# lordnn/OF_DIS

Measured on AMD Instinct MI355X. Metric: MPix/s (and frames/sec) 1080p op-point-2; avg EPE vs CPU ref, higher is better.
Workload: dtype f32; 1 GPU; run_OF_INT 1920x1080 op-point 2, 4096 pairs/GPU/step; width=1920, height=1080, channels=1, oppoint=2, batch_per_gpu=4096, streams=2, pairs_per_launch=2048, parallelism=frame-sharded x1

## Files before the change

### of_dis_amd/csrc/ofdis_internal.h

```cpp
#pragma once

#include <hip/hip_runtime.h>
#include <stdint.h>

namespace ofdis {

struct LevelGeom {
  int w, h;
  int pad;
  int W, H;
  int nopw, noph, npatch, offw, offh;
  float tmp_lb, tmp_ubw, tmp_ubh;
  int level;
};

struct PyrBaseArgs {
  const uint8_t *img_a, *img_b;
  int n, W0, H0, noc;
  int padl, padt;
  int log2s;
  int w, h;
  float *out;
  int rgb_sad;
};

struct PyrGradmagArgs {
  const uint8_t *img_a, *img_b;
  int n, W0, H0, padl, padt, Wp, Hp;
  float *out;
};

struct PyrDownArgs {
  const float *src;
  float *dst;
  int n2, w, h, noc;
};

struct PyrPadGradArgs {
  const float *lvl;
  float *img, *dx, *dy;
  int n2, w, h, noc, pad;
  int per_value;
};

struct PatchArgs {
  const float *img_a, *dx_a, *dy_a, *img_b;
  const float *prev;
  long prev_frame_stride;
  int prev_comp_stride, prev_elem_stride, prev_w;
  float *p_iter;
  float *pweight;
  int n, nop, noc, p, novals, steps;
  int costfct, patnorm, max_iter, min_iter;
  float dp_thresh_sq, dr_thresh, res_thresh, outlierthresh;
  float outlier_sq;
  int camlr;
  int wave_per_patch;
  int generic;
  int window;
  int quad;
  int x16;
  int absw;
  int aslots;
  int buf32;
  int fdiv;
  int maxres;
  int stage;
  LevelGeom g;
};

struct AggArgs {
  const float *p_iter, *pweight;
  const float *cg_p_iter, *cg_pweight;
  float *flow;
  int n, nop, noc, p, novals, steps;
  int absw;
  int aslots;
  int stage;
  LevelGeom g;
};

struct TvArgs {
  const float *img_a, *img_b;
  float *flow;
  float *wxs, *wys;
  float *du, *dv, *mask, *s;
  float *coef;
  float *t, *dt;
  float *Ix, *Iy, *Iz, *Ixx, *Ixy, *Iyy, *Ixz, *Iyz;
  long sp;
  int wrap;
  int skew_slots;
  int n, nop, noc, w, h, pad, W;
  float quarter_alpha, hdo3, hgo3, omega;
  int first_iter;
  int solverit;
  int camlr;
  int sor_generic;
  int sor_variant;
  int sor_point;
  int sor_cring;
  int sor_rows2;
  int smsys;
  int prepd;
  int smsys2d;
  int smsys_prefetch;
  int smsys_small;
  int smsys_march;
  int smsys_deriv;
  int prepd_df;
  int sor_redblack;
  int lat;
};

struct UpArgs {
  const float *flow;
  float *out;
  int n, nop, wl, hl, log2s, W0, H0, offx, offy;
  int nt_store;
  int form;
};

struct InitArgs {
  const float *init;
  float *out;
  int n, nop, W0, H0, padl, padt, log2k, wo, ho;
  float sc, scale;
};

struct FbArgs {
  const float *fw, *bw;
  uint8_t *occ_fw, *occ_bw;
  float *err_fw, *err_bw;
  int n, W, H;
  float alpha, beta;
};

void launch_fb_check(const FbArgs &a, hipStream_t s);
void launch_init_area(const InitArgs &a, hipStream_t s);
void warm_kernels_module(hipStream_t s);
void warm_tvrb_module(hipStream_t s);
void launch_pyr_base(const PyrBaseArgs &a, hipStream_t s);
void launch_pyr_gradmag(const PyrGradmagArgs &a, hipStream_t s);
void launch_pyr_down(const PyrDownArgs &a, hipStream_t s);
void launch_pyr_pad_grad(const PyrPadGradArgs &a, hipStream_t s);
bool launch_patch(const PatchArgs &a, hipStream_t s);
void launch_aggregate(const AggArgs &a, hipStream_t s);
void launch_tv_prep(const TvArgs &a, hipStream_t s);
void launch_tv_deriv1(const TvArgs &a, hipStream_t s);
void launch_tv_deriv2(const TvArgs &a, hipStream_t s);
bool tv_prepd_ok(const TvArgs &a);
void launch_tv_prepd(const TvArgs &a, hipStream_t s);
void launch_tv_smooth(const TvArgs &a, hipStream_t s);
void launch_tv_system(const TvArgs &a, hipStream_t s);
bool tv_smsys_ok(const TvArgs &a);
bool tv_deriv_fused(const TvArgs &a);
void launch_tv_smsys(const TvArgs &a, hipStream_t s);
void launch_tv_sor(const TvArgs &a, hipStream_t s);
bool tv_level_rb_ok(const TvArgs &a);
void launch_tv_level_rb(const TvArgs &a, int n_inner, hipStream_t s);
void launch_tv_final(const TvArgs &a, hipStream_t s);
void launch_upsample(const UpArgs &a, hipStream_t s);

}
```

### of_dis_amd/csrc/ofdis_kernels.hip

```cpp
#include "ofdis_internal.h"
#include "ofdis_math.h"

#include <algorithm>
#include <cstdlib>
#include <type_traits>
#include <utility>

#pragma clang fp contract(off)

namespace ofdis {
typedef float float4_u __attribute__((ext_vector_type(4), aligned(4)));
typedef float float4_v __attribute__((ext_vector_type(4)));

namespace {

#include "ofdis_tv_dev.inc"
#include "ofdis_agg_dev.inc"

inline unsigned ceil_div(long a, long b) { return (unsigned)((a + b - 1) / b); }

template <int V>
using Int = std::integral_constant<int, V>;
template <int... Vs, class F>
inline bool pick(int v, F &&f) {
// ... 3799 lines not shown
      hv[q][s] = nvv[s];
    }
    own_u[q] = cru;
    own_v[q] = crv;
    hsh[q] = csh;
    hsv[q] = csv;
    if (nw > 1) {
      const int par = t & 1;
      float rec[4 * NV4];
#pragma unroll
      for (int s = 0; s < S; ++s) { rec[s] = nu[s]; rec[S + s] = nvv[s]; }
      rec[2 * S] = csv;
#pragma unroll
      for (int k = 2 * S + 1; k < 4 * NV4; ++k) rec[k] = 0.0f;
      if (lane == 63) {
#pragma unroll
        for (int k = 0; k < NV4; ++k) xtop[par][wv][k] = make_float4(rec[4 * k], rec[4 * k + 1], rec[4 * k + 2], rec[4 * k + 3]);
      }
      if (lane == 0) {
#pragma unroll
        for (int k = 0; k < NV4; ++k) xbot[par][wv][k] = make_float4(rec[4 * k], rec[4 * k + 1], rec[4 * k + 2], rec[4 * k + 3]);
      }
      __syncthreads();
    }
  }

  template <int PH>
  __device__ __forceinline__ void steps(const int t) {
    step<PH>(t + PH);
    if constexpr (PH + 1 < U) steps<PH + 1>(t);
  }
};

template <int S, int MODE, int MAXT>
__global__ __launch_bounds__(MAXT) void k_tv_sor_pipe(TvArgs a) {
  using P = SorPipe<S, MODE>;
  __shared__ float4 xtop[2][16][P::NV4];
  __shared__ float4 xbot[2][16][P::NV4];
  P st;
  const int f = blockIdx.x;
  st.w = a.w;
  st.h = a.h;
  st.y = threadIdx.x;
  st.lane = st.y & 63;
  st.wv = st.y >> 6;
  st.nw = (int)(blockDim.x >> 6);
  const long fo = (long)f * a.sp;
  st.du = a.du + fo;
  st.dv = a.dv + fo;
  st.C = reinterpret_cast<const float4 *>(a.coef) + fo * (MODE == 0 ? 2 : 1);
  st.xtop = xtop;
  st.xbot = xbot;
  st.omega = a.omega;
  st.has_top = st.y > 0;
  st.has_bot = st.y < a.h - 1;
  st.notop = !st.has_top;
  st.border = !st.has_top || !st.has_bot;
  st.get_top = st.lane == 0 && st.wv > 0;
  st.get_bot = st.lane == 63 && st.wv < st.nw - 1;
  st.wrap = a.wrap;
  st.dump = (unsigned)(a.skew_slots + st.lane);
#pragma unroll
  for (int q = 0; q < 2; ++q) {
#pragma unroll
    for (int s = 0; s < S; ++s) st.hu[q][s] = st.hv[q][s] = 0.0f;
    st.own_u[q] = st.own_v[q] = st.hsh[q] = st.hsv[q] = 0.0f;
  }
  if (st.y == 0 && a.w > 0) {
    st.own_u[1] = st.du[0];
    if (MODE == 0) st.own_v[1] = st.dv[0];
  }
  const int T = (a.w - 1) + (a.h - 1) + 2 * (S - 1) + 1;
  const int TU = (T + P::U - 1) / P::U * P::U;
  st.load(0, st.L[0]);
  st.load(1, st.L[1]);
  for (int t = 0; t < TU; t += P::U) st.template steps<0>(t);
}

__device__ __forceinline__ int sor_row2(int d, int lim, int rmax) {
  const int dd = max(d, 0);
  return min(dd >= lim ? dd - lim : dd, rmax);
}

template <int S, int MODE, int SI, int NB, int CRN, int R = 1, bool SEL = false>
struct SorLane {
  static constexpr bool FIRST = SI == 0, LAST = SI == S - 1;
  static_assert(CRN == 0 || S <= 3, "coefficient ring depth 6 needs S <= 3");
  static constexpr int PD = NB - 1;
  static constexpr int U = NB % 3 == 0 ? (NB < 6 ? 6 : NB) : 3 * NB;
  static constexpr int CW = MODE == 0 ? 2 : 1;
  struct Ld {
    float4 c0[R], c1[R];
    f2v o[R], b[R];
  };
  Ld L0, L1, L2, L3, L4, L5;
  template <int I>
  __device__ __forceinline__ Ld &buf() {
    static_assert(I < NB && NB <= 6, "buffer index");
    if constexpr (I == 0) return L0;
    else if constexpr (I == 1) return L1;
    else if constexpr (I == 2) return L2;
    else if constexpr (I == 3) return L3;
    else if constexpr (I == 4) return L4;
    else return L5;
  }
  f2v pp[R];
  float phr[R];
  float pvv[R];
  f2v prv[R];
  static constexpr bool DPT = R == 1;
  bool top_lds;
  const float4 *C;
  const float *du_r, *dv_r;
  float *du, *dv;
  f2v *ring_s;
  const f2v *ring_p;
  float *sv_s;
  float4 *cr;
  int w, h, y, s, lim, rmax, hplane;
  unsigned yc[R];
  bool border[R], notop[R];
  float omega;
#ifdef OFDIS_SOR_PROBE
  unsigned *probe = nullptr;
#endif

  __device__ __forceinline__ void load(int t, Ld &B) {
    const int d = t - 2 * s;
    const unsigned r0 = (unsigned)sor_row2(d, lim, rmax) * (unsigned)hplane;
    const unsigned r1 = FIRST ? (unsigned)sor_row2(d + 1, lim, rmax) * (unsigned)hplane : 0u;
#pragma unroll
    for (int r = 0; r < R; ++r) {
      unsigned yr = yc[r];
      if (SEL) {
        const int lo = min(max(d - w + 1, 0), h - 1), hi = max(min(d, h - 1), 0);
        yr = (unsigned)min(max(y + 64 * r, lo), hi);
      }
      if (FIRST || CRN == 0) {
        const float4 *cp = C + (size_t)r0 * CW;
        B.c0[r] = cp[yr * CW];
        if (MODE == 0) B.c1[r] = cp[yr * CW + 1];
      }
      if (FIRST) {
        const float *u0 = du_r + r0, *u1 = du_r + r1;
        float ov = 0.0f, bv = 0.0f;
        if (MODE == 0) {
          const float *v0 = dv_r + r0, *v1 = dv_r + r1;
          ov = v0[yr];
          bv = v1[yr + 1];
        }
        B.o[r] = f2v{u0[yr], ov};
        B.b[r] = f2v{u1[yr + 1], bv};
      }
    }
  }

  template <int Q>
  __device__ __forceinline__ void step(const int t) {
    constexpr int m0 = Q % 3, m1 = (Q + 2) % 3;
#ifdef OFDIS_SOR_PROBE
    const unsigned pt0 = probe_clock();
    unsigned pt1 = 0, pt2 = 0;
#endif
    Ld &B = buf<Q % NB>();
    const Ld &Bn = buf<(Q + 1) % NB>();
    load(t + PD, buf<(Q + PD) % NB>());
    const int d = t - 2 * s;
#pragma unroll
    for (int r = 0; r < R; ++r) {
      constexpr int RO = 64 * 3;
      const int yr = y + 64 * r;
      const int xp = d - yr;
      const bool hasl = xp > 0, hasr = xp < w - 1;
      f2v o, rgt, bt;
      if (FIRST) {
        o = B.o[r]; rgt = Bn.o[r]; bt = B.b[r];
      } else {
        o = prv[r]; rgt = ring_p[r * RO + m1]; bt = ring_p[r * RO + 3 + m1];
        prv[r] = rgt;
      }
      constexpr int cs = ((Q - 2 * SI) % 6 + 6) % 6, ct = (cs + 5) % 6;
      float4 c0, c1;
      if (CRN > 0) {
        if (FIRST) {
          c0 = B.c0[r];
          c1 = MODE == 0 ? B.c1[r] : B.c0[r];
          cr[cs * CW * CRN + 64 * r] = c0;
          if (MODE == 0) cr[(cs * CW + 1) * CRN + 64 * r] = c1;
        } else {
          c0 = cr[cs * CW * CRN + 64 * r];
          c1 = MODE == 0 ? cr[(cs * CW + 1) * CRN + 64 * r] : c0;
        }
      } else {
        c0 = B.c0[r];
        c1 = MODE == 0 ? B.c1[r] : B.c0[r];
      }
      f2v tp;
      float tsv;
      if (DPT) {
        tp = f2v{dpp_from_prev_lane(pp[r].x), MODE == 0 ? dpp_from_prev_lane(pp[r].y) : 0.0f};
        tsv = dpp_from_prev_lane(pvv[r]);
        if (top_lds) {
          tp = ring_s[r * RO + m1 - 3];
          tsv = CRN > 0 ? cr[(ct * CW + CW - 1) * CRN - 1 + 64 * r].w : sv_s[r * RO + m1 - 3];
        }
      } else {
        tp = ring_s[r * RO + m1 - 3];
        tsv = CRN > 0 ? cr[(ct * CW + CW - 1) * CRN - 1 + 64 * r].w : sv_s[r * RO + m1 - 3];
      }
      f2v nw;
      float vv;
#ifdef OFDIS_SOR_PROBE
      {
        const float dep = ((c0.x + c1.x) + (tp.x + tsv)) + (rgt.x + bt.x);
        asm volatile("; probe use %0" ::"v"(dep) : "memory");
        pt1 = probe_clock();
      }
#endif
      if (MODE == 0) {
        const float hr = c1.z;
        vv = c1.w;
        const f2v bb = f2v{c1.x, c1.y};
        const f2v rr = hasr ? rgt : f2v{0.0f, 0.0f};
        const f2v X = hr * rr, Y = tsv * tp, Z = vv * bt;
        const f2v l = X + (border[r] ? bb : Y);
        const f2v rg = (border[r] ? f2v{-0.0f, -0.0f} : bb) + (border[r] ? (notop[r] ? Z : Y) : Z);
        const f2v sr = l + rg;
        const f2v Bv = hasl ? phr[r] * pp[r] + sr : sr;
        const f2v m_1 = f2v{c0.x, c0.y} * Bv.x, m_2 = f2v{c0.z, c0.w} * Bv.y;
        nw = o + omega * ((m_1 + m_2) - o);
        phr[r] = hr;
      } else {
        const float a11 = c0.x, b1 = c0.y, hr = c0.z;
        vv = c0.w;
        const bool has_top = !notop[r], has_bot = !(border[r] && has_top);
        const float tu = tp.x, ur = hasr ? rgt.x : 0.0f, hl = phr[r];
        float su = 0.0f;
        su = has_top ? su - tsv * tu : su;
        su = hasl ? su - hl * pp[r].x : su;
        su = has_bot ? su - vv * bt.x : su;
        su = hasr ? su - hr * ur : su;
        const float A = a11, Bq = b1 - su;
        nw = f2v{(1.0f - omega) * o.x + omega * (Bq / A), 0.0f};
        phr[r] = hr;
      }
      ring_s[r * RO + m0] = nw;
      if (CRN == 0) sv_s[r * RO + m0] = vv;
      pvv[r] = vv;
      if (LAST) {
        if ((unsigned)xp < (unsigned)w && yr < h) {
          const unsigned r0 = (unsigned)sor_row2(d, lim, rmax) * (unsigned)hplane;
          du[r0 + (unsigned)yr] = nw.x;
          if (MODE == 0) dv[r0 + (unsigned)yr] = nw.y;
        }
      }
      pp[r] = nw;
    }
#ifdef OFDIS_SOR_PROBE
    asm volatile("s_waitcnt lgkmcnt(0)" ::: "memory");
    pt2 = probe_clock();
#endif
    __syncthreads();
#ifdef OFDIS_SOR_PROBE
    if (probe && (threadIdx.x & 63) == 0 && t < 1024)
      *reinterpret_cast<uint4 *>(probe + 4 * t) = make_uint4(pt0, pt1, pt2, probe_clock());
#endif
  }

  template <int J>
  __device__ __forceinline__ void prologue(const int t) {
    load(t + J, buf<J>());
    if constexpr (J + 1 < PD) prologue<J + 1>(t);
  }
  template <int J>
  __device__ __forceinline__ void block(const int t) {
    step<J>(t + J);
    if constexpr (J + 1 < U) block<J + 1>(t);
  }

  __device__ __forceinline__ void run(int T, int y0, int ymax) {
#pragma unroll
    for (int r = 0; r < R; ++r) {
      pp[r] = f2v{0.0f, 0.0f};
      phr[r] = 0.0f;
      pvv[r] = 0.0f;
    }
    const int ta = max(0, (y0 + 2 * SI) / U * U);
    const int tb = min(T, (ymax + w - 1 + 2 * SI) / U * U + U);
    for (int t = 0; t < ta; ++t) __syncthreads();
    if (!FIRST) {
#pragma unroll
      for (int r = 0; r < R; ++r) prv[r] = ta >= 2 ? ring_p[64 * 3 * r + (ta - 2) % 3] : f2v{0.0f, 0.0f};
    }
    prologue<0>(ta);
    for (int t = ta; t < tb; t += U) block<0>(t);
    for (int t = tb; t < T; ++t) __syncthreads();
  }
};

constexpr size_t kSorLds = 160 * 1024;
static long device_cus() {
  static long cus[64] = {};
  int dev = 0;
  if (hipGetDevice(&dev) != hipSuccess || dev < 0 || dev >= 64) return 256;
  if (!cus[dev]) {
    int v = 0;
    cus[dev] = hipDeviceGetAttribute(&v, hipDeviceAttributeMultiprocessorCount, dev) == hipSuccess && v > 0 ? v : 256;
  }
  return cus[dev];
}
__host__ __device__ constexpr int sor_crn(int S, int MAXT, int R = 1) {
  return S <= 3 ? 64 * R * (MAXT / (64 * S)) + 2 : 0;
}

__host__ __device__ constexpr size_t sor_cring_bytes(int crn, int cw) { return (size_t)6 * crn * (cw == 2 ? 32 : 16); }
__host__ __device__ __forceinline__ size_t sor_lanes_lds(int S, int h, int crn, int cw, int R = 1) {
  const size_t nr = (size_t)((h + 64 * R - 1) / (64 * R)) * 64 * R + 2;
  const size_t uv = sizeof(float) * 2 * 3 * (size_t)S * nr;
  if (crn == 0) return uv + sizeof(float) * 3 * (size_t)S * nr;
  return (uv + 15) / 16 * 16 + sor_cring_bytes(crn, cw);
}

template <int S, int MODE, int NB, int CRN, int R, bool SEL = false>
__device__ __forceinline__ void sor_lanes_frame(const TvArgs &a, int frame, f2v *ring) {
  constexpr int CW = MODE == 0 ? 2 : 1;
  const int G = (a.h + 64 * R - 1) / (64 * R);
  const int NR = G * 64 * R + 2;
  const int wid = __builtin_amdgcn_readfirstlane(threadIdx.x >> 6), lane = threadIdx.x & 63;
  const int g = wid / S, s = wid - g * S;
  float *svr = reinterpret_cast<float *>(ring + S * 3 * NR);
  char *crb = reinterpret_cast<char *>(ring) + (sizeof(f2v) * S * 3 * NR + 15) / 16 * 16;
  float4 *crr = reinterpret_cast<float4 *>(crb);
  for (int i = threadIdx.x; i < S * 3 * NR; i += blockDim.x) {
    ring[i] = f2v{0.f, 0.f};
    if (CRN == 0) svr[i] = 0.0f;
  }
  if (CRN > 0) {
    float *z = reinterpret_cast<float *>(crb);
    for (int i = threadIdx.x; i < (int)(sor_cring_bytes(CRN, CW) / 4); i += blockDim.x) z[i] = 0.0f;
  }
  __syncthreads();
#ifdef OFDIS_SOR_PROBE
  __shared__ unsigned probe_slot;
  if (threadIdx.x == 0 && frame == 0) probe_slot = g_sor_probe ? atomicAdd(g_sor_probe, 1u) : 64u;
  __syncthreads();
#endif
  const long fo = (long)frame * a.sp;
  constexpr int U = SorLane<S, MODE, 0, NB, CRN, R>::U;
  const int T = ((a.w - 1) + (a.h - 1) + 2 * (S - 1) + 1 + U - 1) / U * U;
  const int y0 = g * 64 * R, ymax = min(y0 + 64 * R - 1, a.h - 1);
  auto setup = [&](auto &st) {
    st.C = reinterpret_cast<const float4 *>(a.coef) + fo * (MODE == 0 ? 2 : 1);
    st.du_r = a.du + fo;
    st.dv_r = a.dv + fo;
    st.du = a.du + fo;
    st.dv = a.dv + fo;
    const int y = y0 + lane;
    st.ring_s = ring + (s * NR + y + 1) * 3;
    st.ring_p = ring + ((s > 0 ? s - 1 : 0) * NR + y + 1) * 3;
    st.sv_s = svr + (s * NR + y + 1) * 3;
    st.cr = crr + y + 1;
    st.w = a.w; st.h = a.h; st.y = y; st.s = s;
    st.lim = a.wrap ? a.w : 1 << 30;
    st.rmax = a.wrap ? a.w - 1 : a.w + a.h - 2;
    st.hplane = a.h;
    st.top_lds = lane == 0 && y0 > 0;
#pragma unroll
    for (int r = 0; r < R; ++r) {
      const int yr = y + 64 * r;
      st.yc[r] = (unsigned)min(yr, a.h - 1);
      st.notop[r] = yr == 0;
      st.border[r] = yr == 0 || yr >= a.h - 1;
    }
    st.omega = a.omega;
#ifdef OFDIS_SOR_PROBE
    if (frame == 0 && probe_slot < 64u && wid < 16)
      st.probe = g_sor_probe + 4 + ((size_t)probe_slot * 16 + wid) * 1024 * 4;
#endif
    st.run(T, y0, ymax);
  };
  if (s == 0) {
    SorLane<S, MODE, 0, NB, CRN, R, SEL> st;
    setup(st);
  } else if (s == 1) {
    SorLane<S, MODE, (S > 1 ? 1 : 0), NB, CRN, R, SEL> st;
    setup(st);
  } else if (s == 2) {
    SorLane<S, MODE, (S > 2 ? 2 : 0), NB, CRN, R, SEL> st;
    setup(st);
  } else {
    SorLane<S, MODE, (S > 3 ? 3 : 0), NB, CRN, R, SEL> st;
    setup(st);
  }
}

template <int S, int MODE, int NB, int MAXT, bool CRING, int R = 1, int CG = 0, bool SEL = false>
__global__ __launch_bounds__(MAXT) void k_tv_sor_lanes(TvArgs a) {
  extern __shared__ f2v ring_uv[];
  constexpr int crn = !CRING ? 0 : CG > 0 ? 64 * R * CG + 2 : sor_crn(S, MAXT, R);
  static_assert(CG == 0 || CG * 64 * S <= MAXT, "row groups of the workgroup");
  sor_lanes_frame<S, MODE, NB, crn, R, SEL>(a, blockIdx.x, ring_uv);
}

}
template <class F>
static void pick_mode(int nop, F &&f) { pick<0, 2>(nop == 2 ? 0 : 2, f); }
template <int S>
static void sor_pipe(const TvArgs &a, hipStream_t s) {
  const int threads = ((a.h + 63) / 64) * 64;
  pick<256, 512, 1024>(threads <= 256 ? 256 : threads <= 512 ? 512 : 1024, [&](auto MAXT) {
    pick_mode(a.nop, [&](auto MODE) { k_tv_sor_pipe<S, MODE, MAXT><<<a.n, threads, 0, s>>>(a); });
  });
}
template <int S, int MAXT, int R>
static bool sor_lanes(const TvArgs &a, hipStream_t s) {
  const int G = (a.h + 64 * R - 1) / (64 * R);
  constexpr int crn = sor_crn(S, MAXT, R);
  const int cw = a.nop == 2 ? 2 : 1;
  const bool cring = crn > 0 && a.sor_cring && sor_lanes_lds(S, a.h, crn, cw, R) <= kSorLds;
  const bool sel = a.sor_cring >= 3 || (long)a.n > device_cus();
  bool launched = false;
  auto go = [&](auto CG, auto CR, size_t lds) {
    if constexpr (!(CR && crn == 0)) {
      pick<0, 1>(sel, [&](auto SEL) {
        pick_mode(a.nop, [&](auto MODE) {
          if constexpr (!(CR && sor_cring_bytes(crn, MODE == 0 ? 2 : 1) > kSorLds)) {
            k_tv_sor_lanes<S, MODE, 3, MAXT, CR != 0, R, CG, SEL != 0><<<a.n, 64 * G * S, lds, s>>>(a);
            launched = true;
          }
        });
      });
    }
  };
  if constexpr (S == 3 && R == 1) {
    if (cring && a.sor_cring >= 2) {
      const size_t ldsg = sor_lanes_lds(S, a.h, 64 * G + 2, cw, R);
      auto ring_g = [&](auto CG) { go(CG, Int<1>{}, ldsg); };
      if constexpr (MAXT == 512) {
        if (pick<1, 2>(G, ring_g)) return launched;
      } else {
        if (pick<3, 4, 5>(G, ring_g)) return launched;
      }
    }
  }
  pick<0, 1>(cring, [&](auto CR) { go(Int<0>{}, CR, sor_lanes_lds(S, a.h, CR ? crn : 0, cw, R)); });
  return launched;
}
template <int S>
static bool sor_lanes_s(const TvArgs &a, hipStream_t s) {
  const int th = 64 * S * ((a.h + 63) / 64);
  if (th <= 512) return sor_lanes<S, 512, 1>(a, s);
  if (th <= 1024) return sor_lanes<S, 1024, 1>(a, s);
  if constexpr (S <= 3) return sor_lanes<S, 1024, 2>(a, s);
  return false;
}
void launch_tv_sor(const TvArgs &a, hipStream_t s) {
  if (a.solverit < 1) return;
  const bool tiny = a.nop == 2 && (a.w < 2 || a.h < 2 || a.sor_point);
  if (a.sor_redblack && !tiny) {
    const dim3 grid(ceil_div(a.w * a.h, 256), a.n);
    pick_mode(a.nop, [&](auto MODE) {
      for (int it = 0; it < 2 * a.solverit; ++it) k_tv_sor_rb<MODE><<<grid, 256, 0, s>>>(a, it & 1);
    });
    return;
  }
  const int G = (a.h + 63) / 64, G2 = (a.h + 127) / 128;
  const bool lanes_fit = G * a.solverit <= 16 || (a.solverit <= 3 && G2 * a.solverit <= 16 && a.sor_rows2);
  bool done = false;
  if (!tiny && !a.sor_generic && a.sor_variant != 1 && lanes_fit)
    pick<2, 3, 4>(a.solverit, [&](auto S) { done = sor_lanes_s<S>(a, s); });
  if (done) return;
  if (!tiny && a.h <= 1024 && !a.sor_generic && pick<1, 2, 3, 4>(a.solverit, [&](auto S) { sor_pipe<S>(a, s); }))
    return;
  pick<0, 1, 2>(a.nop == 1 ? 2 : tiny ? 1 : 0, [&](auto MODE) { k_tv_sor<MODE><<<a.n, 256, 0, s>>>(a); });
}
namespace {

template <int TH>
__global__ __launch_bounds__(256) void k_tv_final(TvArgs a) {
  const uint3 xb = xcd_block();
  __shared__ float sm[2][TH][kTileP];
  constexpr int TD = kTileW + TH - 1;
  const int x0 = xb.x * kTileW, y0 = xb.y * TH, f = xb.z;
  for (int i = threadIdx.x; i < TD * TH; i += 256) {
    const int yy = i & (TH - 1), dd = i / TH, xl = dd - yy;
    const int x = x0 + xl, y = y0 + yy;
    if (xl < 0 || xl >= kTileW || x >= a.w || y >= a.h) continue;
    const long fk = (long)f * a.sp + skw(x, y, a.h, a.w, a.wrap);
    if (a.nop == 2) {
      sm[0][yy][xl] = a.wxs[fk] + a.du[fk];
      sm[1][yy][xl] = a.wys[fk] + a.dv[fk];
    } else {
      const float s = a.wxs[fk] + a.du[fk];
      sm[0][yy][xl] = a.camlr == 0 ? ssemin(s, 0.0f) : ssemax(s, 0.0f);
    }
  }
  __syncthreads();
  const int tx = threadIdx.x & 63, x = x0 + tx;
  const long plane = (long)a.w * a.h;
  float *WX = a.flow + (long)f * a.nop * plane;
  for (int yl = threadIdx.x >> 6; yl < TH; yl += 4) {
    const int y = y0 + yl;
    if (x >= a.w || y >= a.h) continue;
    const long o = (long)y * a.w + x;
    WX[o] = sm[0][yl][tx];
    if (a.nop == 2) WX[plane + o] = sm[1][yl][tx];
  }
}

}
void launch_tv_final(const TvArgs &a, hipStream_t s) {
  k_tv_final<32><<<dim3(ceil_div(a.w, kTileW), ceil_div(a.h, 32), a.n), 256, 0, s>>>(a);
}
namespace {


struct XTap {
  int sx;
  float fx;
  bool lin;
};
__device__ __forceinline__ XTap xtap(int dx, double scale, int wl) {
  XTap r;
  float fx = (float)((dx + 0.5) * scale - 0.5);
  int sx = (int)floorf(fx);
  fx -= (float)sx;
  if (sx < 0) { fx = 0; sx = 0; }
  r.lin = true;
  if (sx + 1 >= wl) {
    r.lin = false;
    if (sx >= wl - 1) { fx = 0; sx = wl - 1; }
  }
// ... 484 lines not shown
```

### of_dis_amd/csrc/ofdis_runtime.cpp

```cpp
#include <hip/hip_runtime.h>

#include <algorithm>
#include <chrono>
#include <cmath>
#include <cstdio>
#include <cstdlib>
#include <cstring>
#include <map>
#include <mutex>
#include <string>
#include <vector>

#include "../../include/ofdis.h"
#include "ofdis_internal.h"

using namespace ofdis;

namespace {

const char *const kKernelNames[] = {"pyr_base", "pyr_down", "pyr_pad_grad", "patch",    "aggregate", "tv_prep",
                                    "tv_deriv", "tv_system", "tv_sor",       "tv_final", "upsample",  "tv_level",
                                    "fb_check", "fb_check_err"};

struct Plan {
  int n = 0, W0 = 0, H0 = 0, Wp = 0, Hp = 0, padl = 0, padt = 0, padw = 0, padh = 0;
  int nop = 2, noc = 1, pad = 8, sc_f = 0, sc_l = 0;
  std::vector<LevelGeom> lv;
  std::vector<size_t> off_lvl, off_img, off_dx, off_dy, off_flow, off_flow_bw;
  size_t off_piter = 0, off_pw = 0, off_piter_bw = 0, off_pw_bw = 0, off_tv = 0, tv_plane = 0;
  size_t off_init = 0;
  bool init = false;
  bool fb = false;
  bool bidir = false;
  size_t off_up_bw = 0;
  bool gradmag = false;
  size_t off_gm = 0;
  size_t total = 0;
};

inline size_t align_up(size_t v) { return (v + 255) & ~(size_t)255; }

inline long skew_plane(int w, int h) {
  const long slots = h <= w ? (long)w * h : (long)(w + h - 1) * h;
  return (slots + 64 + 3) / 4 * 4;
}

}

struct ofdis_context {
  int device = 0;
  hipStream_t stream = nullptr;
  char *ws = nullptr;
  size_t ws_cap = 0;
  std::vector<float *> cap_dis, cap_tv;
  bool timing = false;
  struct Pending {
    int kernel;
    hipEvent_t a, b;
  };
  std::vector<Pending> pending;
  std::vector<hipEvent_t> pool;
  std::map<int, std::pair<double, long>> acc;
  int opt_sor_generic = 0;
  int opt_sor_pipe = 0;
  int opt_graph = 1;
  struct GraphKey {
    const void *a = nullptr, *b = nullptr, *out = nullptr, *ws = nullptr, *init = nullptr;
    const void *flow_bw = nullptr, *occ_fw = nullptr, *occ_bw = nullptr, *err_fw = nullptr, *err_bw = nullptr;
    float alpha = 0.f, beta = 0.f;
    int bidir = 0;
    int n = 0, w = 0, h = 0;
    ofdis_params p{};
  } gkey;
  hipGraphExec_t gexec = nullptr;
  int opt_nt_store = 0;
  int opt_up_form = 3;
  int opt_smsys = 1;
  int opt_smsys2d = 2;
  int opt_smsys_march = 1;
  int opt_smsys_prefetch = 1;
  int opt_smsys_small = 1;
  int opt_agg_stage = 1;
  int opt_pad_grad_v = 1;
  int opt_pyr_rgb = 1;
  int opt_prepd_df = 1;
  int opt_smsys_deriv = 1;
  int call_frames = 1;
  int call_lanes = 1;
  int opt_sor_cring = 2;
  int opt_prepd = 2;
  int opt_sor_rows2 = 1;
  int opt_wave_per_patch = 0;
  int opt_sor_mode = 0;
  int opt_patch_window = 1;
  int opt_patch_quad = 1;
  int opt_patch_x16 = 1;
  int opt_patch_absw = 1;
  int opt_patch_buf = 1;
  int opt_patch_generic = 0;
  int opt_patch_fdiv = 1;
  int opt_patch_maxres = 1;
  int opt_streams = 0, opt_chunk = 0;
  struct Lane {
    hipStream_t s = nullptr;
    char *ws = nullptr;
    size_t cap = 0;
    hipEvent_t done = nullptr;
  };
  std::vector<Lane> lanes;
  hipEvent_t entry = nullptr;
  hipEvent_t ev_null = nullptr, ev_ws = nullptr;
  bool ws_pending = false;
  std::mutex mu;
};

namespace {

bool trace_on() {
  static const bool on = std::getenv("OFDIS_TRACE") && std::getenv("OFDIS_TRACE")[0] == '1';
  return on;
}
#define OFDIS_TRACE(...)                  \
  do {                                    \
    if (trace_on()) {                     \
      std::fprintf(stderr, "ofdis: " __VA_ARGS__); \
      std::fputc('\n', stderr);           \
      std::fflush(stderr);                \
    }                                     \
  } while (0)

#define HIP_OK(x)                                                                                \
  do {                                                                                           \
    hipError_t e_ = (x);                                                                         \
    if (e_ != hipSuccess) {                                                                      \
      std::fprintf(stderr, "ofdis: %s failed: %s (%s:%d)\n", #x, hipGetErrorString(e_), __FILE__, \
                   __LINE__);                                                                    \
      return e_ == hipErrorOutOfMemory ? OFDIS_ERR_OUT_OF_MEMORY : OFDIS_ERR_DEVICE;             \
    }                                                                                            \
  } while (0)

int kernel_index(const char *name) {
  for (int i = 0; i < (int)(sizeof(kKernelNames) / sizeof(kKernelNames[0])); ++i)
    if (std::strcmp(kKernelNames[i], name) == 0) return i;
  return -1;
}

hipEvent_t get_event(ofdis_context *c) {
  if (!c->pool.empty()) {
    hipEvent_t e = c->pool.back();
    c->pool.pop_back();
    return e;
  }
  hipEvent_t e = nullptr;
  if (hipEventCreate(&e) != hipSuccess) return nullptr;
  return e;
}

template <class F>
void timed(ofdis_context *c, int kernel, hipStream_t s, F &&f) {
  if (!c->timing) {
    f();
    return;
  }
  hipEvent_t a = get_event(c), b = get_event(c);
  hipEventRecord(a, s);
  f();
  hipEventRecord(b, s);
  c->pending.push_back({kernel, a, b});
}

void drain_timing(ofdis_context *c) {
  for (auto &p : c->pending) {
// ... 231 lines not shown
    }
    bool absw = false;
    timed(c, 3, s, [&] { absw = launch_patch(pa, s); });
    PatchArgs pb = pa;
    const bool bw = P.fb || P.bidir;
    bool absw_bw = false;
    if (bw) {
      pb.img_a = img + (size_t)n * fsp;
      pb.dx_a = dxp + (size_t)n * fsp;
      pb.dy_a = dyp + (size_t)n * fsp;
      pb.img_b = img;
      pb.prev = nullptr;
      if (sl < p->sc_f) pb.prev = (const float *)(ws + P.off_flow_bw[i + 1]);
      pb.p_iter = (float *)(ws + P.off_piter_bw);
      pb.pweight = (float *)(ws + P.off_pw_bw);
      pb.camlr = 1;
      timed(c, 3, s, [&] { absw_bw = launch_patch(pb, s); });
    }

    AggArgs ag{};
    ag.p_iter = pa.p_iter;
    ag.pweight = pa.pweight;
    ag.flow = flow;
    ag.n = n;
    ag.nop = nop;
    ag.noc = noc;
    ag.p = p->p_samp_s;
    ag.novals = novals;
    ag.absw = absw;
    ag.aslots = pa.aslots;
    ag.stage = c->opt_agg_stage;
    ag.steps = steps;
    ag.g = g;
    ag.cg_p_iter = P.fb ? pb.p_iter : nullptr;
    ag.cg_pweight = P.fb ? pb.pweight : nullptr;
    float *flow_bw = (float *)(ws + P.off_flow_bw[i]);
    const int n_inner = p->tv_innerit * (sl + 1);
    auto make_tv = [&](int dir) {
      const long sp = skew_plane(g.w, g.h);
      const size_t pl = (size_t)n * sp;
      float *t0 = (float *)(ws + P.off_tv);
      TvArgs tv{};
      tv.img_a = dir == 0 ? img : img + (size_t)n * fsp;
      tv.img_b = dir == 0 ? img + (size_t)n * fsp : img;
      tv.flow = dir == 0 ? flow : flow_bw;
      tv.du = t0;
      tv.dv = t0 + pl;
      tv.mask = t0 + 2 * pl;
      tv.coef = t0 + 3 * pl;
      tv.s = t0 + 11 * pl;
      tv.wxs = t0 + 12 * pl;
      tv.wys = t0 + 13 * pl;
      tv.sp = sp;
      tv.wrap = g.h <= g.w;
      tv.skew_slots = tv.wrap ? g.w * g.h : (g.w + g.h - 1) * g.h;
      float *cp = t0 + 14 * pl;
      const size_t cpl = pl * noc;
      tv.t = cp;
      tv.dt = cp + cpl;
      tv.Iz = tv.dt;
      tv.Ix = cp + 2 * cpl;
      tv.Iy = cp + 3 * cpl;
      tv.Ixx = cp + 4 * cpl;
      tv.Ixy = cp + 5 * cpl;
      tv.Iyy = cp + 6 * cpl;
      tv.Ixz = cp + 7 * cpl;
      tv.Iyz = cp + 8 * cpl;
      tv.n = n;
      tv.nop = nop;
      tv.noc = noc;
      tv.w = g.w;
      tv.h = g.h;
      tv.pad = g.pad;
      tv.W = g.W;
      tv.quarter_alpha = 0.25f * p->tv_alpha;
      tv.hgo3 = p->tv_gamma * 0.5f / 3.0f;
      tv.hdo3 = p->tv_delta * 0.5f / 3.0f;
      tv.omega = p->tv_sor;
      tv.solverit = p->tv_solverit;
      tv.camlr = dir;
      tv.sor_generic = c->opt_sor_generic;
      tv.sor_variant = c->opt_sor_pipe;
      tv.sor_cring = c->opt_sor_cring;
      tv.sor_rows2 = c->opt_sor_rows2;
      tv.smsys = c->opt_smsys;
      tv.smsys2d = c->opt_smsys2d == 2 ? c->call_frames < 512 : c->opt_smsys2d;
      tv.smsys_march = c->opt_smsys_march;
      tv.smsys_prefetch = c->opt_smsys_prefetch;
      tv.smsys_small = c->opt_smsys_small;
      tv.smsys_deriv = c->opt_smsys_deriv;
      tv.prepd_df = c->opt_prepd_df;
      tv.sor_redblack = c->opt_sor_mode == 1;
      tv.sor_point = p->omp_build && nop == 2;
      tv.prepd = c->opt_prepd;
      return tv;
    };
    if (times) HIP_OK(hipEventRecord(ev[3], s));
    timed(c, 4, s, [&] { launch_aggregate(ag, s); });
    const bool bw_level = bw && (sl > p->sc_l || P.bidir);
    if (bw_level) {
      AggArgs ab = ag;
      ab.p_iter = pb.p_iter;
      ab.pweight = pb.pweight;
      ab.cg_p_iter = P.fb ? pa.p_iter : nullptr;
      ab.cg_pweight = P.fb ? pa.pweight : nullptr;
      ab.absw = absw_bw;
      ab.flow = flow_bw;
      timed(c, 4, s, [&] { launch_aggregate(ab, s); });
    }
    if (times) HIP_OK(hipEventRecord(ev[4], s));
    int rc = capture(c, s, c->cap_dis, sl, P, flow);
    if (rc) return rc;

    for (int dir = 0; dir < (bw_level ? 2 : 1) && p->usetvref && n_inner > 0; ++dir) {
      TvArgs tv = make_tv(dir);
      tv.lat = tv_level_rb_ok(tv);
      tv.smsys_deriv = !tv.lat && tv_deriv_fused(tv);
      if (tv_prepd_ok(tv)) {
        timed(c, 5, s, [&] { launch_tv_prepd(tv, s); });
      } else {
        timed(c, 5, s, [&] { launch_tv_prep(tv, s); });
        timed(c, 6, s, [&] {
          launch_tv_deriv1(tv, s);
          launch_tv_deriv2(tv, s);
        });
      }
      if (tv.lat) {
        timed(c, 11, s, [&] { launch_tv_level_rb(tv, n_inner, s); });
        continue;
      }
      for (int it = 0; it < n_inner; ++it) {
        tv.first_iter = it == 0;
        timed(c, 7, s, [&] {
          if (tv_smsys_ok(tv)) {
            launch_tv_smsys(tv, s);
          } else {
            launch_tv_smooth(tv, s);
            launch_tv_system(tv, s);
          }
        });
        timed(c, 8, s, [&] { launch_tv_sor(tv, s); });
      }
      timed(c, 9, s, [&] { launch_tv_final(tv, s); });
    }
    if (times) {
      HIP_OK(hipEventRecord(ev[5], s));
      HIP_OK(hipEventSynchronize(ev[5]));
      StageTimes st;
      float t01, t12, t23, t34, t45;
      hipEventElapsedTime(&t01, ev[0], ev[1]);
      hipEventElapsedTime(&t12, ev[1], ev[2]);
      hipEventElapsedTime(&t23, ev[2], ev[3]);
      hipEventElapsedTime(&t34, ev[3], ev[4]);
      hipEventElapsedTime(&t45, ev[4], ev[5]);
      st.pconst = t01;
      st.pinit = std::max(0.0, (double)t12 - t01);
      st.poptim = std::max(0.0, (double)t23 - t12);
      st.cflow = t34;
      st.tvopt = t45;
      times->push_back(st);
    }
    rc = capture(c, s, c->cap_tv, sl, P, flow);
    if (rc) return rc;
  }
  if (times)
    for (auto &e : ev) hipEventDestroy(e);
  return hipGetLastError() == hipSuccess ? OFDIS_OK : OFDIS_ERR_DEVICE;
// ... 629 lines not shown
      for (int k = 0; k < 4; ++k)
        if (host_f[k]) step(hipMemcpy(host_f[k], d + off_f[k], bytes_f[k], hipMemcpyDeviceToHost));
      for (int k = 0; k < 2; ++k)
        if (host_u[k]) step(hipMemcpy(host_u[k], d + off_u[k], px, hipMemcpyDeviceToHost));
    }
  }
  hipFree(d);
  return rc;
}

int ofdis_pyramid_u8_host(ofdis_context *c, const uint8_t *img, int width, int height, const ofdis_params *p,
                          int imgpadding, float *const *img_pyr, float *const *dx_pyr, float *const *dy_pyr) {
  if (!c || !img || !p || width <= 0 || height <= 0) return OFDIS_ERR_INVALID_ARGUMENT;
  std::lock_guard<std::mutex> lock(c->mu);
  HIP_OK(hipSetDevice(c->device));
  ofdis_params q = *p;
  q.p_samp_s = imgpadding;
  Plan P = batch_plan(p, 1, width, height);
  P = make_plan(p, 1, P.Wp, P.Hp, imgpadding);
  {
    const int d = 1 << p->sc_f;
    P.W0 = width;
    P.H0 = height;
    P.padw = (width % d) ? d - width % d : 0;
    P.padh = (height % d) ? d - height % d : 0;
    P.padl = P.padw / 2;
    P.padt = P.padh / 2;
  }
  int rc = ensure_ws(c, P.total);
  if (rc) return rc;
  const size_t in = (size_t)width * height * p->noc;
  uint8_t *d = nullptr;
  HIP_OK(hipMalloc(&d, in));
  HIP_OK(hipMemcpy(d, img, in, hipMemcpyHostToDevice));
  hipStream_t st;
  rc = call_begin(c, c->stream, st);
  if (rc == OFDIS_OK) rc = run_pyramid(c, c->ws, P, d, d, st);
  if (rc == OFDIS_OK) rc = call_end(c, c->stream, st);
  if (rc == OFDIS_OK) {
    HIP_OK(hipStreamSynchronize(c->stream));
    for (int s = p->sc_l; s <= p->sc_f; ++s) {
      const LevelGeom &g = P.lv[s - p->sc_l];
      const size_t bytes = sizeof(float) * (size_t)g.W * g.H * p->noc;
      if (img_pyr && img_pyr[s]) HIP_OK(hipMemcpy(img_pyr[s], c->ws + P.off_img[s - p->sc_l], bytes, hipMemcpyDeviceToHost));
      if (dx_pyr && dx_pyr[s]) HIP_OK(hipMemcpy(dx_pyr[s], c->ws + P.off_dx[s - p->sc_l], bytes, hipMemcpyDeviceToHost));
      if (dy_pyr && dy_pyr[s]) HIP_OK(hipMemcpy(dy_pyr[s], c->ws + P.off_dy[s - p->sc_l], bytes, hipMemcpyDeviceToHost));
    }
  }
  hipFree(d);
  (void)q;
  return rc;
}

int ofdis_context_set_stage_capture(ofdis_context *c, float *const *dis_flow, float *const *tv_flow, int nscales) {
  if (!c || nscales < 0) return OFDIS_ERR_INVALID_ARGUMENT;
  std::lock_guard<std::mutex> lock(c->mu);
  c->cap_dis.assign(nscales, nullptr);
  c->cap_tv.assign(nscales, nullptr);
  bool any = false;
  for (int i = 0; i < nscales; ++i) {
    if (dis_flow) c->cap_dis[i] = dis_flow[i];
    if (tv_flow) c->cap_tv[i] = tv_flow[i];
    any = any || c->cap_dis[i] || c->cap_tv[i];
  }
  if (!any) {
    c->cap_dis.clear();
    c->cap_tv.clear();
  }
  return OFDIS_OK;
}

int ofdis_context_set_option(ofdis_context *c, const char *key, int value) {
  if (!c || !key) return OFDIS_ERR_INVALID_ARGUMENT;
  std::lock_guard<std::mutex> lock(c->mu);
  struct Opt {
    const char *name;
    int ofdis_context::*field;
    int lo, hi;
  };
  static const Opt opts[] = {
      {"sor_generic", &ofdis_context::opt_sor_generic, 0, 1},
      {"sor_pipe", &ofdis_context::opt_sor_pipe, 0, 1},     {"smsys", &ofdis_context::opt_smsys, 0, 1},
      {"sor_cring", &ofdis_context::opt_sor_cring, 0, 3},   {"smsys2d", &ofdis_context::opt_smsys2d, 0, 2},
      {"smsys_march", &ofdis_context::opt_smsys_march, 0, 1},
      {"smsys_prefetch", &ofdis_context::opt_smsys_prefetch, 0, 1},
      {"smsys_small", &ofdis_context::opt_smsys_small, 0, 1},
      {"smsys_deriv", &ofdis_context::opt_smsys_deriv, 0, 1},
      {"prepd_df", &ofdis_context::opt_prepd_df, 0, 1},
      {"pyr_rgb", &ofdis_context::opt_pyr_rgb, 0, 1},
      {"pad_grad_v", &ofdis_context::opt_pad_grad_v, 0, 1},
      {"agg_stage", &ofdis_context::opt_agg_stage, 0, 1},
      {"sor_rows2", &ofdis_context::opt_sor_rows2, 0, 1},   {"prepd", &ofdis_context::opt_prepd, 0, 2},
      {"wave_per_patch", &ofdis_context::opt_wave_per_patch, 0, 1},
      {"nt_store", &ofdis_context::opt_nt_store, 0, 1},     {"up_form", &ofdis_context::opt_up_form, 0, 3},
      {"graph", &ofdis_context::opt_graph, 0, 2},
      {"patch_window", &ofdis_context::opt_patch_window, 0, 1}, {"patch_quad", &ofdis_context::opt_patch_quad, 0, 1},
      {"patch_generic", &ofdis_context::opt_patch_generic, 0, 1}, {"sor_mode", &ofdis_context::opt_sor_mode, 0, 1},
      {"patch_x16", &ofdis_context::opt_patch_x16, 0, 2},  {"patch_absw", &ofdis_context::opt_patch_absw, 0, 1},
      {"patch_buf", &ofdis_context::opt_patch_buf, 0, 1},  {"patch_fdiv", &ofdis_context::opt_patch_fdiv, 0, 1},
      {"patch_maxres", &ofdis_context::opt_patch_maxres, 0, 1},
      {"streams", &ofdis_context::opt_streams, 0, 16},      {"chunk", &ofdis_context::opt_chunk, 0, 1 << 30},
  };
  for (const Opt &o : opts) {
    if (std::strcmp(key, o.name) != 0) continue;
    if (value < o.lo || value > o.hi) return OFDIS_ERR_INVALID_ARGUMENT;
    HIP_OK(hipSetDevice(c->device));
    const int rc = drop_graph(c);
    if (rc) return rc;
    c->*o.field = (o.hi == 1) ? (value != 0) : value;
    return OFDIS_OK;
  }
  return OFDIS_ERR_INVALID_ARGUMENT;
}

int ofdis_context_enable_kernel_timing(ofdis_context *c, int enable) {
  if (!c) return OFDIS_ERR_INVALID_ARGUMENT;
  std::lock_guard<std::mutex> lock(c->mu);
  drain_timing(c);
  c->acc.clear();
  c->timing = enable != 0;
  return OFDIS_OK;
}

int ofdis_context_kernel_time(ofdis_context *c, const char *name, double *total_ms, long *launches) {
  if (!c || !name) return OFDIS_ERR_INVALID_ARGUMENT;
  const int k = kernel_index(name);
  if (k < 0) return OFDIS_ERR_INVALID_ARGUMENT;
  std::lock_guard<std::mutex> lock(c->mu);
  drain_timing(c);
  auto it = c->acc.find(k);
  if (total_ms) *total_ms = it == c->acc.end() ? 0.0 : it->second.first;
  if (launches) *launches = it == c->acc.end() ? 0 : it->second.second;
  return OFDIS_OK;
}

const char *ofdis_kernel_names(void) {
  static const std::string names = [] {
    std::string r;
    for (const char *k : kKernelNames) r += (r.empty() ? "" : ",") + std::string(k);
    return r;
  }();
  return names.c_str();
}

int ofdis_algorithmic_bytes(const ofdis_params *p, int width, int height, const char *kernel, double *bytes) {
  if (!p || !kernel || !bytes) return OFDIS_ERR_INVALID_ARGUMENT;
  Plan P = batch_plan(p, 1, width, height);
  const int nop = P.nop, noc = P.noc;
  const int novals = noc * p->p_samp_s * p->p_samp_s;
  double b = 0.0;
  const std::string k(kernel);
  if (("," + std::string(ofdis_kernel_names()) + ",").find("," + k + ",") == std::string::npos)
    return OFDIS_ERR_INVALID_ARGUMENT;
  for (const LevelGeom &g : P.lv) {
    const double px = (double)g.w * g.h;
    const int n_inner = p->usetvref ? p->tv_innerit * (g.level + 1) : 0;
    if (k == "tv_sor") b += n_inner * p->tv_solverit * px * (nop == 2 ? 44.0 : 24.0);
    if (k == "tv_level" && n_inner > 0) b += px * 4.0 * (2 * nop + 8 * noc);
    if (k == "tv_system") b += n_inner * px * (4.0 * (8 * noc + 1 + 2 * nop) + 4.0 * (nop == 2 ? 7 : 4));
    if (k == "patch") b += (double)g.npatch * (12.0 * novals + 4.0 * (p->p_samp_s + 1) * (p->p_samp_s + 1) * noc +
                                               4.0 * (nop + novals));
    if (k == "aggregate") b += px * 4.0 * nop + (double)g.npatch * 4.0 * (nop + novals);
    if (k == "pyr_pad_grad") b += 2.0 * (px * 4.0 * noc + 3.0 * g.W * g.H * 4.0 * noc);
    if (k == "pyr_down" && g.level > p->sc_l) b += 2.0 * noc * 4.0 * (4.0 * px + px);
    if (p->usetvref) {
      if (k == "tv_prep") b += px * 4.0 * (4 * noc + 1 + 3 * nop);
      if (k == "tv_deriv") b += px * 4.0 * noc * (2 + 4 + 2 + 3);
// ... 86 lines not shown
```

Baseline: 328,000 MPix/s.

## Pack multiple small-level frames into one SOR workgroup

Adds a packed SOR lanes kernel that stacks F frames vertically within one workgroup when the pyramid level height is small (at most 128 rows). Each lane maps its virtual row to a frame offset and local row, and stores are masked by a per-lane liveness flag. The aim is to stop small coarse levels from leaving most of a 64-wide wave and workgroup idle, and to cut the number of workgroups. In exchange it uses more LDS and threads per workgroup, and needs extra index arithmetic per lane.

```diff
diff --git a/of_dis_amd/csrc/ofdis_internal.h b/of_dis_amd/csrc/ofdis_internal.h
--- a/of_dis_amd/csrc/ofdis_internal.h
+++ b/of_dis_amd/csrc/ofdis_internal.h
@@ -100,6 +100,7 @@
   int sor_variant;
   int sor_point;
   int sor_cring;
+  int sor_pack;
   int sor_rows2;
   int smsys;
   int prepd;
diff --git a/of_dis_amd/csrc/ofdis_kernels.hip b/of_dis_amd/csrc/ofdis_kernels.hip
--- a/of_dis_amd/csrc/ofdis_kernels.hip
+++ b/of_dis_amd/csrc/ofdis_kernels.hip
@@ -3905,9 +3905,10 @@
   return min(dd >= lim ? dd - lim : dd, rmax);
 }
 
-template <int S, int MODE, int SI, int NB, int CRN, int R = 1, bool SEL = false>
+template <int S, int MODE, int SI, int NB, int CRN, int R = 1, bool SEL = false, bool PK = false>
 struct SorLane {
   static constexpr bool FIRST = SI == 0, LAST = SI == S - 1;
+  static_assert(!PK || R == 1, "packed frames run one row per lane");
   static_assert(CRN == 0 || S <= 3, "coefficient ring depth 6 needs S <= 3");
   static constexpr int PD = NB - 1;
   static constexpr int U = NB % 3 == 0 ? (NB < 6 ? 6 : NB) : 3 * NB;
@@ -3942,6 +3943,8 @@
   float4 *cr;
   int w, h, y, s, lim, rmax, hplane;
   unsigned yc[R];
+  unsigned fo;
+  bool live;
   bool border[R], notop[R];
   float omega;
 #ifdef OFDIS_SOR_PROBE
@@ -3958,6 +3961,7 @@
       if (SEL) {
         const int lo = min(max(d - w + 1, 0), h - 1), hi = max(min(d, h - 1), 0);
         yr = (unsigned)min(max(y + 64 * r, lo), hi);
+        if (PK) yr += fo;
       }
       if (FIRST || CRN == 0) {
         const float4 *cp = C + (size_t)r0 * CW;
@@ -4071,10 +4075,11 @@
       if (CRN == 0) sv_s[r * RO + m0] = vv;
       pvv[r] = vv;
       if (LAST) {
-        if ((unsigned)xp < (unsigned)w && yr < h) {
+        if ((unsigned)xp < (unsigned)w && (PK ? live : yr < h)) {
           const unsigned r0 = (unsigned)sor_row2(d, lim, rmax) * (unsigned)hplane;
-          du[r0 + (unsigned)yr] = nw.x;
-          if (MODE == 0) dv[r0 + (unsigned)yr] = nw.y;
+          const unsigned ys = PK ? fo + (unsigned)yr : (unsigned)yr;
+          du[r0 + ys] = nw.x;
+          if (MODE == 0) dv[r0 + ys] = nw.y;
         }
       }
       pp[r] = nw;
@@ -4144,10 +4149,10 @@
   return (uv + 15) / 16 * 16 + sor_cring_bytes(crn, cw);
 }
 
-template <int S, int MODE, int NB, int CRN, int R, bool SEL = false>
-__device__ __forceinline__ void sor_lanes_frame(const TvArgs &a, int frame, f2v *ring) {
+template <int S, int MODE, int NB, int CRN, int R, bool SEL = false, bool PK = false>
+__device__ __forceinline__ void sor_lanes_frame(const TvArgs &a, int frame, f2v *ring, int F = 1) {
   constexpr int CW = MODE == 0 ? 2 : 1;
-  const int G = (a.h + 64 * R - 1) / (64 * R);
+  const int G = ((PK ? F * a.h : a.h) + 64 * R - 1) / (64 * R);
   const int NR = G * 64 * R + 2;
   const int wid = __builtin_amdgcn_readfirstlane(threadIdx.x >> 6), lane = threadIdx.x & 63;
   const int g = wid / S, s = wid - g * S;
@@ -4171,27 +4176,39 @@
   const long fo = (long)frame * a.sp;
   constexpr int U = SorLane<S, MODE, 0, NB, CRN, R>::U;
   const int T = ((a.w - 1) + (a.h - 1) + 2 * (S - 1) + 1 + U - 1) / U * U;
-  const int y0 = g * 64 * R, ymax = min(y0 + 64 * R - 1, a.h - 1);
+  int y0 = g * 64 * R, ymax = min(y0 + 64 * R - 1, a.h - 1);
+  const int v0 = y0;
+  const int nf = min(F, a.n - frame);
+  if (PK) {
+    const int v1 = min(v0 + 63, nf * a.h - 1);
+    const int f0 = v0 / a.h, f1 = v1 / a.h;
+    y0 = v1 < v0 ? 0 : f0 == f1 ? v0 - f0 * a.h : 0;
+    ymax = v1 < v0 ? 0 : f0 == f1 ? v1 - f0 * a.h : a.h - 1;
+  }
   auto setup = [&](auto &st) {
     st.C = reinterpret_cast<const float4 *>(a.coef) + fo * (MODE == 0 ? 2 : 1);
     st.du_r = a.du + fo;
     st.dv_r = a.dv + fo;
     st.du = a.du + fo;
     st.dv = a.dv + fo;
-    const int y = y0 + lane;
-    st.ring_s = ring + (s * NR + y + 1) * 3;
-    st.ring_p = ring + ((s > 0 ? s - 1 : 0) * NR + y + 1) * 3;
-    st.sv_s = svr + (s * NR + y + 1) * 3;
-    st.cr = crr + y + 1;
+    const int v = v0 + lane;
+    const int fl = PK ? v / a.h : 0;
+    const int y = v - fl * a.h;
+    st.ring_s = ring + (s * NR + v + 1) * 3;
+    st.ring_p = ring + ((s > 0 ? s - 1 : 0) * NR + v + 1) * 3;
+    st.sv_s = svr + (s * NR + v + 1) * 3;
+    st.cr = crr + v + 1;
     st.w = a.w; st.h = a.h; st.y = y; st.s = s;
+    st.live = fl < nf;
+    st.fo = (unsigned)min(fl, nf - 1) * (unsigned)a.sp;
     st.lim = a.wrap ? a.w : 1 << 30;
     st.rmax = a.wrap ? a.w - 1 : a.w + a.h - 2;
     st.hplane = a.h;
-    st.top_lds = lane == 0 && y0 > 0;
+    st.top_lds = lane == 0 && v0 > 0 && y > 0;
 #pragma unroll
     for (int r = 0; r < R; ++r) {
       const int yr = y + 64 * r;
-      st.yc[r] = (unsigned)min(yr, a.h - 1);
+      st.yc[r] = PK ? st.fo + (unsigned)y : (unsigned)min(yr, a.h - 1);
       st.notop[r] = yr == 0;
       st.border[r] = yr == 0 || yr >= a.h - 1;
     }
@@ -4203,16 +4220,16 @@
     st.run(T, y0, ymax);
   };
   if (s == 0) {
-    SorLane<S, MODE, 0, NB, CRN, R, SEL> st;
+    SorLane<S, MODE, 0, NB, CRN, R, SEL, PK> st;
     setup(st);
   } else if (s == 1) {
-    SorLane<S, MODE, (S > 1 ? 1 : 0), NB, CRN, R, SEL> st;
+    SorLane<S, MODE, (S > 1 ? 1 : 0), NB, CRN, R, SEL, PK> st;
     setup(st);
   } else if (s == 2) {
-    SorLane<S, MODE, (S > 2 ? 2 : 0), NB, CRN, R, SEL> st;
+    SorLane<S, MODE, (S > 2 ? 2 : 0), NB, CRN, R, SEL, PK> st;
     setup(st);
   } else {
-    SorLane<S, MODE, (S > 3 ? 3 : 0), NB, CRN, R, SEL> st;
+    SorLane<S, MODE, (S > 3 ? 3 : 0), NB, CRN, R, SEL, PK> st;
     setup(st);
   }
 }
@@ -4223,6 +4240,13 @@
   constexpr int crn = !CRING ? 0 : CG > 0 ? 64 * R * CG + 2 : sor_crn(S, MAXT, R);
   static_assert(CG == 0 || CG * 64 * S <= MAXT, "row groups of the workgroup");
   sor_lanes_frame<S, MODE, NB, crn, R, SEL>(a, blockIdx.x, ring_uv);
+}
+template <int S, int MODE, int NB, int MAXT, int CG, bool SEL>
+__global__ __launch_bounds__(MAXT) void k_tv_sor_lanes_pack(TvArgs a, int F) {
+  extern __shared__ f2v ring_uv[];
+  constexpr int crn = CG > 0 ? 64 * CG + 2 : sor_crn(S, MAXT, 1);
+  static_assert(CG == 0 || CG * 64 * S <= MAXT, "row groups of the workgroup");
+  sor_lanes_frame<S, MODE, NB, crn, 1, SEL, true>(a, blockIdx.x * F, ring_uv, F);
 }
 
 }
@@ -4269,8 +4293,50 @@
   pick<0, 1>(cring, [&](auto CR) { go(Int<0>{}, CR, sor_lanes_lds(S, a.h, CR ? crn : 0, cw, R)); });
   return launched;
 }
+constexpr int kSorPackGroups = 4;
+static int sor_pack_frames(const TvArgs &a, int S) {
+  if (!a.sor_pack || !a.sor_cring || S > 3 || a.h < 2 || a.h > 128) return 0;
+  if (a.sor_pack < 2 && (long)a.n <= device_cus()) return 0;
+  const int F = 64 * kSorPackGroups / a.h, G = (F * a.h + 63) / 64, G1 = (a.h + 63) / 64;
+  if (F < 2 || G * S > 16 || 4 * G > 3 * G1 * F) return 0;
+  if ((long)F * a.sp * 32 >= (1L << 31)) return 0;
+  return F;
+}
+template <int S>
+static bool sor_lanes_pack(const TvArgs &a, hipStream_t s) {
+  if constexpr (S > 3) {
+    return false;
+  } else {
+    const int F = sor_pack_frames(a, S);
+    if (!F) return false;
+    const int G = (F * a.h + 63) / 64, cw = a.nop == 2 ? 2 : 1;
+    const bool sel = a.sor_cring >= 3 || (long)a.n > device_cus();
+    const int wgs = (a.n + F - 1) / F;
+    bool launched = false;
+    auto go = [&](auto MAXT, auto CG) {
+      const int crn = CG > 0 ? 64 * CG + 2 : sor_crn(S, MAXT, 1);
+      const size_t lds = sor_lanes_lds(S, F * a.h, crn, cw, 1);
+      if (lds > kSorLds) return;
+      pick<0, 1>(sel, [&](auto SEL) {
+        pick_mode(a.nop, [&](auto MODE) {
+          k_tv_sor_lanes_pack<S, MODE, 3, MAXT, CG, SEL != 0><<<wgs, 64 * G * S, lds, s>>>(a, F);
+          launched = true;
+        });
+      });
+    };
+    if constexpr (S == 3) {
+      if (G <= 2) pick<1, 2>(G, [&](auto CG) { go(Int<512>{}, CG); });
+      else pick<3, 4, 5>(G, [&](auto CG) { go(Int<1024>{}, CG); });
+    } else {
+      if (G <= 4) go(Int<512>{}, Int<0>{});
+      else go(Int<1024>{}, Int<0>{});
+    }
+    return launched;
+  }
+}
 template <int S>
 static bool sor_lanes_s(const TvArgs &a, hipStream_t s) {
+  if (sor_lanes_pack<S>(a, s)) return true;
   const int th = 64 * S * ((a.h + 63) / 64);
   if (th <= 512) return sor_lanes<S, 512, 1>(a, s);
   if (th <= 1024) return sor_lanes<S, 1024, 1>(a, s);
diff --git a/of_dis_amd/csrc/ofdis_runtime.cpp b/of_dis_amd/csrc/ofdis_runtime.cpp
--- a/of_dis_amd/csrc/ofdis_runtime.cpp
+++ b/of_dis_amd/csrc/ofdis_runtime.cpp
@@ -88,6 +88,7 @@
   int call_frames = 1;
   int call_lanes = 1;
   int opt_sor_cring = 2;
+  int opt_sor_pack = 1;
   int opt_prepd = 2;
   int opt_sor_rows2 = 1;
   int opt_wave_per_patch = 0;
@@ -485,7 +486,7 @@
       tv.sor_generic = c->opt_sor_generic;
       tv.sor_variant = c->opt_sor_pipe;
       tv.sor_cring = c->opt_sor_cring;
-      tv.sor_rows2 = c->opt_sor_rows2;
+      tv.sor_pack = c->opt_sor_pack;      tv.sor_rows2 = c->opt_sor_rows2;
       tv.smsys = c->opt_smsys;
       tv.smsys2d = c->opt_smsys2d == 2 ? c->call_frames < 512 : c->opt_smsys2d;
       tv.smsys_march = c->opt_smsys_march;
@@ -1281,7 +1282,7 @@
       {"sor_generic", &ofdis_context::opt_sor_generic, 0, 1},
       {"sor_pipe", &ofdis_context::opt_sor_pipe, 0, 1},     {"smsys", &ofdis_context::opt_smsys, 0, 1},
       {"sor_cring", &ofdis_context::opt_sor_cring, 0, 3},   {"smsys2d", &ofdis_context::opt_smsys2d, 0, 2},
-      {"smsys_march", &ofdis_context::opt_smsys_march, 0, 1},
+      {"sor_pack", &ofdis_context::opt_sor_pack, 0, 2},      {"smsys_march", &ofdis_context::opt_smsys_march, 0, 1},
       {"smsys_prefetch", &ofdis_context::opt_smsys_prefetch, 0, 1},
       {"smsys_small", &ofdis_context::opt_smsys_small, 0, 1},
       {"smsys_deriv", &ofdis_context::opt_smsys_deriv, 0, 1},
```

New measurement: 342,100 MPix/s (median of 6 runs). +4.3%, better.
